# supernomad/quantum

Measured on AMD Instinct MI355X. Metric: AES-256-GCM seal+unseal GiB/s (device-resident packets) at 1/2/4/8 MI355X, higher is better.
Workload: dtype u8

## Files before the change

### quantum_amd/csrc/gcm_kernels.hip

```cpp
#include <hip/hip_runtime.h>
#include <stdint.h>

#include <algorithm>

#include "gcm_internal.h"

namespace qgcm {

typedef __attribute__((address_space(3))) uint32_t lds_u32;
typedef uint32_t u32x4 __attribute__((ext_vector_type(4)));
typedef __attribute__((address_space(3))) u32x4 lds_u128;

struct __attribute__((aligned(4))) W4 {
    uint32_t x, y, z, w;
};

#ifndef QGCM_NT_DATA
#define QGCM_NT_DATA 0
#endif
typedef uint32_t u32x4u __attribute__((ext_vector_type(4), aligned(4)));
__device__ __forceinline__ W4 load_block(const W4 *p) {
    if constexpr ((QGCM_NT_DATA & 1) != 0) {
        const u32x4u v = __builtin_nontemporal_load(reinterpret_cast<const u32x4u *>(p));
        return W4{v.x, v.y, v.z, v.w};
// ... 415 lines not shown
__device__ __forceinline__ void write_tail(uint8_t *data, uint32_t L, uint32_t g0, uint32_t g1, uint32_t g2,
                                           uint32_t g3, uint32_t n0, uint32_t n1, uint32_t n2, uint32_t prefix) {
    const uint32_t s = L & 3u;
    uint32_t *t = reinterpret_cast<uint32_t *>(data + (L & ~3u));
    const uint32_t sh = 32 - 8 * s;
    t[0] = (uint32_t)((((uint64_t)g0 << 32) | ((uint64_t)prefix << sh)) >> sh);
    t[1] = funnel(g1, g0, sh);
    t[2] = funnel(g2, g1, sh);
    t[3] = funnel(g3, g2, sh);
    t[4] = funnel(n0, g3, sh);
    t[5] = funnel(n1, n0, sh);
    t[6] = funnel(n2, n1, sh);
    if (s) store_bytes(data + (L & ~3u) + 28, n2 >> sh, s);
}

__device__ __forceinline__ uint32_t quad_xor(uint32_t v) {
    v ^= (uint32_t)__builtin_amdgcn_mov_dpp((int)v, 0xB1, 0xf, 0xf, false);
    v ^= (uint32_t)__builtin_amdgcn_mov_dpp((int)v, 0x4E, 0xf, 0xf, false);
    return v;
}

template <bool kSeal, class Eng>
__device__ __forceinline__ void quad_packet(const Batch &b, const Eng &eng, uint32_t pkt, uint64_t off, uint32_t L,
                                            uint32_t wkey, uint32_t m, uint32_t gH4) {
    const uint4 *Hg = b.gh_table + (size_t)wkey * kGhEntries;
    uint8_t *raw = b.arena + off;
    uint8_t *data = raw + 4;

    uint32_t g0 = 0, g1 = 0, g2 = 0, g3 = 0, n0, n1, n2;
    if (kSeal && b.nonces) {
        const uint32_t *np = reinterpret_cast<const uint32_t *>(b.nonces + 12ull * pkt);
        n0 = np[0];
        n1 = np[1];
        n2 = np[2];
    } else {
        read_nonce(data, L, n0, n1, n2);
    }
    const uint32_t nfull = L >> 4, r = L & 15u;
    const uint32_t d = nfull + (r ? 1u : 0u);

    uint32_t z0 = 0, z1 = 0, z2 = 0, z3 = 0;
    if (m == 3 && b.aad_len)
        z0 = *reinterpret_cast<const uint32_t *>(raw) & (b.aad_len >= 4 ? 0xffffffffu : lowmask(b.aad_len));
    int blast = -1;

    uint32_t e0 = 0, e1 = 0, e2 = 0, e3 = 0;
    uint32_t prefix = 0;
    {
    Ctr cc;
    uint32_t hi = 0;
    eng.setup(cc, n0, n1, n2, 0);
    for (uint32_t bi = m; bi < nfull; bi += 4) {
        const uint32_t ctr = bi + 2;
        if ((ctr >> 8) != hi) {
            hi = ctr >> 8;
            eng.setup(cc, n0, n1, n2, hi);
        }
        W4 *p = reinterpret_cast<W4 *>(data + 16u * bi);
        const W4 in = load_block(p);
        uint32_t k0, k1, k2, k3;
        eng.block(cc, ctr & 0xffu, k0, k1, k2, k3);
        const W4 out = {in.x ^ k0, in.y ^ k1, in.z ^ k2, in.w ^ k3};
        store_block(p, out);
        const W4 &c = kSeal ? out : in;
        eng.ghash(z0, z1, z2, z3, gH4);
        z0 ^= c.x;
        z1 ^= c.y;
        z2 ^= c.z;
        z3 ^= c.w;
        blast = (int)bi;
    }
    const bool part = r && (nfull & 3u) == m;
    if (part || m == (d & 3u)) {
        const uint32_t ctr = part ? nfull + 2 : 1u;
        if ((ctr >> 8) != hi) {
            hi = ctr >> 8;
            eng.setup(cc, n0, n1, n2, hi);
        }
        uint32_t k0, k1, k2, k3;
        eng.block(cc, ctr & 0xffu, k0, k1, k2, k3);
        if (part) {
            uint8_t *blk = data + 16u * nfull;
            const W4 in = *reinterpret_cast<const W4 *>(blk);
            const uint32_t q = r >> 2, sb = r & 3u;
            const uint32_t o0 = in.x ^ k0, o1 = in.y ^ k1, o2 = in.z ^ k2, o3 = in.w ^ k3;
            uint32_t *bw = reinterpret_cast<uint32_t *>(blk);
            if (q > 0) bw[0] = o0;
            if (q > 1) bw[1] = o1;
            if (q > 2) bw[2] = o2;
            const uint32_t oq = sel4(q, o0, o1, o2, o3) & lowmask(sb);
            W4 c = kSeal ? W4{o0, o1, o2, o3} : in;
            if (kSeal)
                prefix = oq;
            else
                store_bytes(blk + 4 * q, oq, sb);
            c.x &= q > 0 ? 0xffffffffu : lowmask(sb);
            c.y &= q > 1 ? 0xffffffffu : (q == 1 ? lowmask(sb) : 0u);
            c.z &= q > 2 ? 0xffffffffu : (q == 2 ? lowmask(sb) : 0u);
            c.w &= q == 3 ? lowmask(sb) : 0u;
            eng.ghash(z0, z1, z2, z3, gH4);
            z0 ^= c.x;
            z1 ^= c.y;
            z2 ^= c.z;
            z3 ^= c.w;
            blast = (int)nfull;
        } else {
            e0 = k0;
            e1 = k1;
            e2 = k2;
            e3 = k3;
        }
    }
    }
    {
        const uint32_t em = d + 1u - (uint32_t)blast;
        const uint32_t tsel = em == 2 ? kGhH2 : em == 3 ? kGhH3 : em == 4 ? kGhH4 : kGhH5;
        ghash_mul_global(z0, z1, z2, z3, Hg + tsel);
        uint32_t l0, l1, l2, l3;
        ghash_lenblock_global(b.aad_len, L, Hg, l0, l1, l2, l3);
        z0 = quad_xor(z0) ^ l0;
        z1 = quad_xor(z1) ^ l1;
        z2 = quad_xor(z2) ^ l2;
        z3 = quad_xor(z3) ^ l3;
    }
    e0 = quad_xor(e0);
    e1 = quad_xor(e1);
    e2 = quad_xor(e2);
    e3 = quad_xor(e3);
    const uint32_t t0 = z0 ^ e0, t1 = z1 ^ e1, t2 = z2 ^ e2, t3 = z3 ^ e3;
    const uint32_t owner = r ? (nfull & 3u) : 0u;
    if (kSeal) {
        if (m == owner) {
            write_tail(data, L, t0, t1, t2, t3, n0, n1, n2, prefix);
            if (b.status) b.status[pkt] = 1;
        }
    } else {
        read_tag(data, L, g0, g1, g2, g3);
        const bool ok = ((t0 ^ g0) | (t1 ^ g1) | (t2 ^ g2) | (t3 ^ g3)) == 0;
        if (!ok) {
            for (uint32_t bi = m; bi < nfull; bi += 4) {
                const W4 zz = {0, 0, 0, 0};
                *reinterpret_cast<W4 *>(data + 16u * bi) = zz;
            }
            if (r && m == owner) {
                uint32_t *bw = reinterpret_cast<uint32_t *>(data + 16u * nfull);
                for (uint32_t w = 0; w < (r >> 2); ++w) bw[w] = 0;
                store_bytes(data + 16u * nfull + (r & ~3u), 0, r & 3u);
            }
        }
        if (b.status && m == 0) b.status[pkt] = ok ? 1 : 0;
    }
}

#ifndef QGCM_TILE_POOL
#define QGCM_TILE_POOL 4
#endif
#ifndef QGCM_TAIL_EIGHTHS
#define QGCM_TAIL_EIGHTHS 4
#endif
constexpr uint32_t kPoolCtr = kG5Bytes + kTeBytes;

#ifdef QGCM_QUAD_STATS
__device__ unsigned long long g_quad_stats[4096 * 8];
#endif

template <bool kDesc>
constexpr int quad_waves() { return kDesc ? 12 : 16; }
template <bool kDesc>
constexpr int quad_wpe() { return kDesc ? 3 : 8; }

template <bool kSeal, bool kDesc>
__global__ void __launch_bounds__(quad_waves<kDesc>() * 64) __attribute__((amdgpu_waves_per_eu(quad_wpe<kDesc>(),
                                                                                                  quad_wpe<kDesc>())))
gcm_quad_kernel(Batch b, const uint32_t *__restrict__ rk_table) {
    constexpr uint32_t kW = quad_waves<kDesc>();
    constexpr uint32_t kT = kW * 64;
    constexpr uint32_t kTeBase = kDesc ? 0u : kG5Bytes;
    const uint32_t lane = threadIdx.x & 63u;
    const uint32_t wave = threadIdx.x >> 6;
    const uint32_t m = lane & 3u;
    const uint32_t qd = lane >> 2;
    if (kDesc && b.tile_list && __builtin_amdgcn_readfirstlane(*b.n_list) == 0) return;

    for (uint32_t i = threadIdx.x; i < kTeBytes / 4; i += kT) {
        const uint32_t x = i >> 6, slot = i & 63u;
        lds_st32(kTeBase + 4 * i, b.te[(slot >> 5) * 256u + x]);
    }
    if constexpr (!kDesc) g5_fill(b.gh_table + (size_t)b.uniform_key * kGhEntries + kGhH4, threadIdx.x, kT);
    if constexpr (!kDesc && QGCM_TILE_POOL) {
        if (threadIdx.x == 0) lds_st32(kPoolCtr, kW);
    }
#if QGCM_TILE_POOL == 4
    if constexpr (!kDesc) {
        if (threadIdx.x == 0) lds_st32(kPoolCtr + 12, 0u);
    }
#endif
    __syncthreads();

    const uint32_t lb = (lane & 31u) << 2;
    const uint32_t m8 = vreg(0x0000ff00u), mf8 = vreg(0x000000f8u);
    const uint32_t gH4 = kDesc ? kTeBytes + wave * kGhBytes : 0u;
    uint32_t cur_key = kDesc ? 0xffffffffu : b.uniform_key;
    const uint32_t ntiles = kDesc ? (b.tile_list ? *b.n_list : b.n_items >> 4) : ((b.n + 15) >> 4);

#ifdef QGCM_QUAD_STATS
    unsigned long long *qs = g_quad_stats + (size_t)blockIdx.x * 8u;
    uint32_t qs_tiles = 0;
    if (!kDesc && threadIdx.x == 0) {
        qs[0] = wall_clock64();
        qs[4] = __builtin_amdgcn_s_getreg((31 << 11) | 20);
        qs[5] = __builtin_amdgcn_s_getreg((31 << 11) | 4);
    }
#endif
#ifdef QGCM_QUAD_STATS
#define QS_TILE() ++qs_tiles
#define QS_END()                                                  \
    do {                                                          \
        if (!kDesc && lane == 0) {                                \
            const unsigned long long t_ = wall_clock64();         \
            atomicMax(&qs[1], t_);                                \
            atomicAdd(&qs[2], t_);                                \
            atomicAdd(&qs[3], (unsigned long long)qs_tiles);      \
            atomicMax(&qs[6], (1ull << 62) - t_);                 \
        }                                                         \
    } while (0)
#else
#define QS_TILE() do { } while (0)
#define QS_END() do { } while (0)
#endif
#if QGCM_TILE_POOL == 4
    uint32_t sidx = 0xffffffffu, tail0 = 0;
    if constexpr (!kDesc) {
        const uint32_t rows = ntiles / (gridDim.x * kW);
        if (b.pool && rows > 0) {
            const uint32_t tail_rows = rows < 2 ? 0u : std::min(rows - 1u, std::max(1u, rows * QGCM_TAIL_EIGHTHS / 8u));
            sidx = (rows - tail_rows) * kW;
            tail0 = (rows - tail_rows) * gridDim.x * kW;
        }
    }
#endif
    uint32_t tile = blockIdx.x * kW + wave;
    if constexpr (kDesc) {
        uint32_t t = 0;
        if (lane == 0) t = atomicAdd(b.tile_counter, 1u);
        tile = __builtin_amdgcn_readfirstlane(__shfl(t, 0));
    }
    for (; tile < ntiles;) {
        uint32_t pkt, L;
        bool valid;
        uint64_t off;
        uint32_t wkey = cur_key;
        if constexpr (kDesc) {
            const uint32_t wt = b.tile_list ? b.tile_list[tile] : tile;
            pkt = b.worklist[wt * 16u + qd];
            valid = pkt != 0xffffffffu;
            qgcm_desc dsc = {0, 0, 0};
            if (valid) dsc = b.descs[pkt];
            off = dsc.offset;
            L = kSeal ? dsc.len : dsc.len - QGCM_OVERHEAD;
            const uint64_t vmask = __ballot(valid);
            if (vmask != 0) {
                wkey = __builtin_amdgcn_readfirstlane(__shfl(dsc.key_idx, __ffsll((unsigned long long)vmask) - 1));
                if (wkey != cur_key) {
                    const uint4 *src = b.gh_table + (size_t)wkey * kGhEntries + kGhH4;
#pragma unroll
                    for (int r = 0; r < 8; ++r) {
                        const uint32_t e = r * 64 + lane;
                        lds_st_comb(gH4, e, src[e]);
                    }
                    __builtin_amdgcn_fence(__ATOMIC_RELEASE, "wavefront");
                    __builtin_amdgcn_wave_barrier();
                    __builtin_amdgcn_fence(__ATOMIC_ACQUIRE, "wavefront");
                    cur_key = wkey;
                }
            }
            uint32_t t = 0;
            if (lane == 0) t = atomicAdd(b.tile_counter, 1u);
            const uint32_t next = __builtin_amdgcn_readfirstlane(__shfl(t, 0));
            asm volatile("" : "+v"(L));
            if (!valid) {
                tile = next;
                continue;
            }
            tile = next;
        } else {
            pkt = tile * 16u + qd;
            L = b.uniform_len;
            asm volatile("" : "+s"(L));
            valid = pkt < b.n;
            if (!kSeal) {
                if (L < (uint32_t)QGCM_OVERHEAD) valid = false;
                L -= QGCM_OVERHEAD;
            }
            off = (uint64_t)pkt * b.stride;
            if constexpr (QGCM_TILE_POOL) {
                uint32_t i = 0;
                if (lane == 0) i = __atomic_fetch_add((lds_u32 *)(size_t)kPoolCtr, 1u, __ATOMIC_RELAXED);
                i = __builtin_amdgcn_readfirstlane(i);
                tile = blockIdx.x * kW + (i % kW) + (i / kW) * gridDim.x * kW;
#if QGCM_TILE_POOL == 4
                if (i >= sidx) {
                    uint32_t c = 0;
                    if (lane == 0) c = atomicAdd(b.pool, 1u);
                    tile = tail0 + __builtin_amdgcn_readfirstlane(c);
                }
#endif
            } else {
                tile += gridDim.x * kW;
            }
            if (!valid) {
                if (!kSeal && b.status && pkt < b.n && m == 0) b.status[pkt] = 0;
                continue;
            }
        }
        const Keys kk = {rk_table + (size_t)wkey * kRkWords, rk_table + (size_t)wkey * kRkWords + 64};
        if constexpr (kDesc) {
            quad_packet<kSeal>(b, Tab2{kk, {lb, m8}}, pkt, off, L, wkey, m, gH4);
        } else {
            quad_packet<kSeal>(b, Tab2F{kk, {lb, m8}, mf8}, pkt, off, L, wkey, m, gH4);
        }
        QS_TILE();
    }
    QS_END();
#if QGCM_TILE_POOL == 4
    if constexpr (!kDesc) {
        if (b.pool) {
            uint32_t last = 0;
            if (lane == 0 && __atomic_fetch_add((lds_u32 *)(size_t)(kPoolCtr + 12), 1u, __ATOMIC_RELAXED) == kW - 1) {
                __threadfence();
                last = atomicAdd(b.pool + kPoolDoneWord, 1u) == gridDim.x - 1u ? 1u : 0u;
            }
            if (lane == 0 && last) {
                __threadfence();
                b.pool[0] = 0;
                b.pool[kPoolDoneWord] = 0;
                __threadfence_system();
                __hip_atomic_store(b.pool_done, b.pool_gen, __ATOMIC_RELEASE, __HIP_MEMORY_SCOPE_SYSTEM);
            }
        }
    }
#endif
}
#undef QS_TILE
#undef QS_END

#ifdef QGCM_QUAD_STATS
extern "C" int qgcm_debug_quad_stats(unsigned long long *out, int n, int reset) {
    if (n > 4096 * 8) n = 4096 * 8;
    if (hipMemcpyFromSymbol(out, HIP_SYMBOL(g_quad_stats), (size_t)n * 8) != hipSuccess) return -1;
    if (reset) {
        static unsigned long long zero[4096 * 8];
        if (hipMemcpyToSymbol(HIP_SYMBOL(g_quad_stats), zero, sizeof(zero)) != hipSuccess) return -1;
    }
    return 0;
}
#endif

constexpr uint32_t kSegCtl = kG5Bytes + kTeBytes;
constexpr uint32_t kSegLds = kSegCtl + 16u;
constexpr uint32_t kSegDone = 0xffffffffu;

__device__ __forceinline__ volatile lds_u32 *seg_ctl(uint32_t i) { return (volatile lds_u32 *)(size_t)(kSegCtl + 4u * i); }

template <class P>
__device__ __forceinline__ uint32_t wave_lower_bound(uint32_t lo, uint32_t hi, uint32_t lane, P pred) {
    while (hi - lo > 63u) {
        const uint32_t step = (hi - lo + 62u) / 63u;
        const uint32_t p = min(lo + lane * step, hi);
        const uint64_t msk = __ballot(pred(p));
        const uint32_t f = (uint32_t)__ffsll((unsigned long long)msk) - 1u;
        if (f == 0) return lo;
        const uint32_t nlo = lo + (f - 1u) * step + 1u, nhi = min(lo + f * step, hi);
        lo = nlo;
        hi = nhi;
    }
    const uint64_t msk = __ballot(pred(min(lo + lane, hi)));
    return lo + (uint32_t)__ffsll((unsigned long long)msk) - 1u;
}

#ifdef QGCM_SEG_STATS
__device__ unsigned long long g_seg_stats[4096 * 16];
#define SEG_STAT_ADD(i, v) \
    do { if (lane == 0) atomicAdd(&g_seg_stats[blockIdx.x * 16u + (i)], (unsigned long long)(v)); } while (0)
#define SEG_NOW() wall_clock64()
#else
#define SEG_STAT_ADD(i, v) do { } while (0)
#define SEG_NOW() 0ull
#endif

#ifndef QGCM_SEG_START
#define QGCM_SEG_START 1
#endif
#ifndef QGCM_SEG_HELP_MIN
#define QGCM_SEG_HELP_MIN 16
#endif
#ifndef QGCM_SEG_LAST
#define QGCM_SEG_LAST 0
#endif
__device__ __forceinline__ void seg_next_phase(const Batch &b, uint32_t &r, uint32_t nruns, bool &helping,
                                               uint32_t lane) {
    uint32_t found = kSegDone;
    if (!helping) {
        uint32_t c = 0;
        if (lane == 0) c = atomicAdd(b.tile_counter, 1u);
        c = __builtin_amdgcn_readfirstlane(__shfl(c, 0));
        if (c < nruns)
            found = c;
        else
            helping = true;
    }
    if (helping) {
        if (QGCM_SEG_START) {
            const uint32_t h = (blockIdx.x * 0x9E3779B1u) ^ (r * 0x85EBCA6Bu + 0x632BE5ABu);
            r = (uint32_t)(((uint64_t)(h ^ (h >> 15)) * nruns) >> 32);
        }
        for (uint32_t pass = 0, need = QGCM_SEG_HELP_MIN; pass < (QGCM_SEG_LAST ? 2u : 1u) && found == kSegDone;
             ++pass, need = QGCM_SEG_LAST ? QGCM_SEG_LAST : 1u)
        for (uint32_t base = 0; base < nruns; base += 256u) {
            bool left[4];
            uint32_t idx[4];
#pragma unroll
            for (uint32_t j = 0; j < 4; ++j) {
                const uint32_t o = base + 64u * j + lane;
                uint32_t i = r + o;
                i = i >= nruns ? i - nruns : i;
                idx[j] = i;
                left[j] = false;
                if (o < nruns) {
                    const uint2 run = b.runs[i];
                    left[j] = __hip_atomic_load(b.run_next + i, __ATOMIC_RELAXED, __HIP_MEMORY_SCOPE_AGENT) +
                                  need <= run.y - run.x;
                }
            }
#pragma unroll
            for (uint32_t j = 0; j < 4 && found == kSegDone; ++j) {
                const uint64_t msk = __ballot(left[j]);
                if (msk) found = __builtin_amdgcn_readfirstlane(__shfl(idx[j], (int)__ffsll((unsigned long long)msk) - 1));
            }
            if (found != kSegDone) break;
        }
    }
    uint32_t key = kSegDone;
    if (found != kSegDone) {
        r = found;
        key = b.tile_keys[b.runs[found].x];
    }
    if (lane == 0) {
        *seg_ctl(0) = found;
        *seg_ctl(1) = key;
    }
}

#ifndef QGCM_SEG_CLAIM
#define QGCM_SEG_CLAIM 1
#endif

template <bool kSeal>
__global__ void __launch_bounds__(1024) __attribute__((amdgpu_waves_per_eu(8, 8)))
gcm_seg_kernel(Batch b, const uint32_t *__restrict__ rk_table) {
    constexpr uint32_t kT = 1024;
    const uint32_t lane = threadIdx.x & 63u;
    const uint32_t wave = threadIdx.x >> 6;
    const uint32_t m = lane & 3u;
    const uint32_t qd = lane >> 2;
    if (__builtin_amdgcn_readfirstlane(*b.nruns) == 0) return;
    for (uint32_t i = threadIdx.x; i < kTeBytes / 4; i += kT) {
        const uint32_t x = i >> 6, slot = i & 63u;
        lds_st32(kG5Bytes + 4 * i, b.te[(slot >> 5) * 256u + x]);
    }
    const uint32_t lb = (lane & 31u) << 2;
    const uint32_t m8 = vreg(0x0000ff00u), mf8 = vreg(0x000000f8u);
    const uint32_t ntiles = b.n_items >> 4;
    uint32_t table_key = kSegDone;
    uint32_t r = 0, nruns = 0;
// ... 1274 lines not shown
```

### quantum_amd/csrc/qgcm_api.cpp

```cpp
#include <hip/hip_runtime.h>
#include <errno.h>
#include <stdint.h>
#include <stdio.h>
#include <stdlib.h>
#include <string.h>
#include <sys/random.h>

#include <algorithm>
#include <atomic>
#include <chrono>
#include <memory>
#include <future>
#include <map>
#include <mutex>
#include <thread>
#include <vector>

#include "../../include/qgcm.h"
#include "chain_claim.h"
#include "gcm_internal.h"
#include "kdf_core.h"

using namespace qgcm;

constexpr int kPipeStreams = 3;
constexpr uint64_t kPipeChunk = 32ull << 20;
constexpr uint64_t kHostChunk = 64ull << 20;
constexpr uint64_t kHostRing = 4ull << 30;

struct qgcm_ctx {
    int device = 0;
    int num_cus = 0;
    uint32_t max_keys = 0;
    int uniform_variant = kVariantUniform;
    int desc_variant = kVariantDescQuad;
    int wgs_per_cu_override = 0;
    bool one_kernel = true;
    bool variant_forced = false;
    uint32_t desc_one_max = kDescOneMax;
    uint32_t direct_max = kDirectMax;
    uint32_t one_uniform_max = kOneUniformMax;
    uint32_t launch_chunk = kLaunchChunk;
    uint32_t desc_chunk = kDescChunk;
    bool desc_one_on = true, host_direct = true, small_wl = true;
    uint64_t chain_chunk = kPipeChunk;
    int chain_slots = kPipeStreams, chain_dev_ahead = 2, chain_dev_backlog = -1;
    bool snappy_group = true;
    int snappy_per_cu = 0;
    bool chain_pin = true;
    std::mutex codec_cpus_mu;
    std::vector<int> codec_cpus;
    uint32_t *d_rk = nullptr;
    uint4 *d_gh = nullptr;
    uint4 *d_pw = nullptr;
    uint32_t pw_keys = 0;
    uint32_t *d_te = nullptr;
    uint8_t *d_sbox = nullptr;
    uint8_t *d_key_valid = nullptr;
    std::vector<uint8_t> key_set;
    std::mutex key_mu;

    std::mutex ws_mu;
    void *d_qws = nullptr;
    size_t qws_cap = 0;

    std::mutex io_mu;
    struct OneSlot {
        std::mutex mu;
        hipStream_t stream = nullptr;
        uint8_t *h = nullptr;
        size_t cap = 0;
    };
    static constexpr int kOneSlots = 8;
    static constexpr size_t kOneSlotCap = kOneCap + 4096;
    static_assert((kOneCap - 16u) + 16u <= kOneSlotCap, "record, tail and status bytes fit a pooled staging slot");
    static_assert(one_fits_launch(16336, true, QGCM_MAX_AAD) && !one_fits_launch(16337, true, QGCM_MAX_AAD) &&
                      one_record_bytes(16336, true) + one_tail_bytes(QGCM_MAX_AAD) + 16u <= kOneSlotCap,
                  "the largest long-AAD call fits a pooled staging slot");
    OneSlot one[kOneSlots];
    OneSlot big;
    std::atomic<uint32_t> one_rr{0};

    hipStream_t pipe[kPipeStreams] = {};
    std::vector<hipEvent_t> ev_in, ev_kern, ev_out;
    uint64_t host_chunk = kHostChunk, host_ring = kHostRing;
    uint8_t *d_ring = nullptr;
    size_t ring_cap = 0;
    uint8_t *h_stat = nullptr;
    size_t hstat_cap = 0;
    uint8_t *d_side = nullptr;
    size_t side_cap = 0;
    qgcm_desc *h_desc = nullptr;
    uint32_t *h_lens = nullptr;
    std::vector<hipStream_t> chain_extra;
    size_t hdesc_cap = 0;

    hipEvent_t ws_done = nullptr;
    bool ws_pending = false;

    uint32_t *d_pool = nullptr;
    uint32_t *h_pool_done = nullptr;
    uint32_t pool_gen[kPoolSets] = {};
    uint32_t pool_launches = 0;
    uint32_t pool_sets = kPoolSets;
    std::mutex pool_mu;

    qgcm::NonceRng rng;

    std::atomic<uint64_t> launches[QGCM_KERNEL_COUNTERS] = {};
    void count(int k, uint64_t v = 1) { launches[k].fetch_add(v, std::memory_order_relaxed); }

    std::atomic<int> chain_codec{1};

    bool res_on = true;
    qgcm::ResidentConfig res_cfg{};
    std::atomic<qgcm::Resident *> res{nullptr};
    std::atomic<bool> res_failed{false};
    std::mutex res_mu;

    uint32_t kdf_device_min = kKdfDeviceMin;
    std::mutex kdf_mu;
    hipStream_t kdf_stream = nullptr;
    std::atomic<uint64_t> kdf_stats[4] = {};
    std::atomic<uint64_t> ecdh_stats[3] = {};

    qgcm::RouteState *route = nullptr;
};

namespace {

thread_local bool tl_dummy;

int env_int(const char *name, int dflt) {
    const char *v = getenv(name);
    return v && *v ? atoi(v) : dflt;
}

uint8_t gf8_mul(uint8_t a, uint8_t b) {
    uint8_t p = 0;
    for (int i = 0; i < 8; ++i) {
        if (b & 1) p ^= a;
        const uint8_t hi = a & 0x80;
        a <<= 1;
        if (hi) a ^= 0x1b;
        b >>= 1;
    }
    return p;
}

void build_tables(uint8_t sbox[256], uint32_t te[512]) {
    for (int x = 0; x < 256; ++x) {
        uint8_t inv = 0;
        if (x) {
            uint8_t r = 1, b = (uint8_t)x;
            for (int e = 254; e; e >>= 1) {
                if (e & 1) r = gf8_mul(r, b);
                b = gf8_mul(b, b);
            }
            inv = r;
        }
        auto rl = [](uint8_t v, int s) { return (uint8_t)((v << s) | (v >> (8 - s))); };
        sbox[x] = inv ^ rl(inv, 1) ^ rl(inv, 2) ^ rl(inv, 3) ^ rl(inv, 4) ^ 0x63;
    }
    for (int x = 0; x < 256; ++x) {
        const uint32_t s = sbox[x], s2 = gf8_mul((uint8_t)s, 2), s3 = s2 ^ s;
        const uint32_t t0 = s2 | (s << 8) | (s << 16) | (s3 << 24);
        te[x] = t0;
        te[256 + x] = (t0 << 8) | (t0 >> 24);
    }
}

void set_err(char *err, int errlen, const char *msg) {
    if (err && errlen > 0) snprintf(err, (size_t)errlen, "%s", msg);
}

int hip_fail(hipError_t e) { return e == hipSuccess ? QGCM_OK : QGCM_E_HIP; }

int grid_for(const qgcm_ctx *ctx, uint32_t n_items, int variant) {
    const int cus = std::max(1, ctx->num_cus - resident_workers_running(ctx->res.load(std::memory_order_acquire)));
    const uint32_t waves = (uint32_t)variant_waves(variant);
    const uint32_t tiles = (n_items + 15) / 16;
    const uint32_t wgs = (tiles + waves - 1) / waves;
    const uint32_t per_cu = ctx->wgs_per_cu_override > 0 ? (uint32_t)ctx->wgs_per_cu_override
                                                         : (uint32_t)variant_wgs_per_cu(variant);
    const uint32_t cap = (uint32_t)cus * per_cu;
    return (int)(wgs < cap ? (wgs ? wgs : 1) : cap);
}

Batch base_batch(const qgcm_ctx *ctx) {
    Batch b{};
    b.rk_table = ctx->d_rk;
    b.gh_table = ctx->d_gh;
    b.pw_table = ctx->d_pw;
    b.pw_keys = ctx->pw_keys;
    b.te = ctx->d_te;
    b.key_valid = ctx->d_key_valid;
    b.max_keys = ctx->max_keys;
    return b;
}

int run_uniform(qgcm_ctx *ctx, bool seal, uint8_t *arena, uint64_t stride, uint32_t n, uint32_t len,
                uint32_t key_idx, const uint8_t *nonces, uint32_t aad_len, uint8_t *status, hipStream_t s,
                const NonceLease *lease = nullptr, uint64_t lease_pos = 0);

inline bool generate(const uint8_t *nonces) { return nonces == QGCM_NONCES_GENERATE; }

int nonce_launch(qgcm_ctx *ctx, NonceDest dest, const NonceLease &l, uint8_t *out, const qgcm_desc *descs,
                 uint64_t stride, uint32_t len, uint32_t n, bool one, hipStream_t s) {
    NonceArgs a{};
    a.keys = l.keys;
    a.v0 = l.v[0];
    a.v1 = l.v[1];
    a.v2 = l.v[2];
    a.v3 = l.v[3];
    a.out = out;
    a.descs = descs;
    a.key_valid = ctx->d_key_valid;
    a.te = ctx->d_te;
    a.stride = stride;
    a.len = len;
    a.n = n;
    a.max_keys = ctx->max_keys;
    a.one = one ? 1u : 0u;
    return hip_fail(launch_nonce_fill(dest, a, ctx->num_cus, s));
}

int run_one(qgcm_ctx *ctx, bool seal, uint8_t *slot, uint64_t stride, uint32_t len, uint32_t key_idx,
            uint32_t aad_len, uint8_t *status, hipStream_t s) {
    if (ctx->one_kernel && stride + one_tail_bytes(aad_len) <= kOneCap - 16 && !(stride & 15) &&
        !((uintptr_t)slot & 15)) {
        volatile uint8_t *done = status + 1;
        *done = 0;
        Batch b = base_batch(ctx);
        b.done = status + 1;
        b.arena = slot;
        b.status = status;
        b.stride = stride;
        b.uniform_len = len;
        b.uniform_key = key_idx;
        b.n = 1;
        b.n_items = 64;
        b.aad_len = aad_len;
        if (launch_one(seal, b, s) != hipSuccess) return QGCM_E_HIP;
        ctx->count(QGCM_KERNEL_ONE);
        const auto t0 = std::chrono::steady_clock::now();
        for (uint32_t spins = 0; *done == 0; ++spins) {
            __builtin_ia32_pause();
            if ((spins & 1023) == 1023 && std::chrono::steady_clock::now() - t0 > std::chrono::seconds(1)) break;
        }
        if (*done == 0) return hip_fail(hipStreamSynchronize(s));
        std::atomic_thread_fence(std::memory_order_acquire);
        return QGCM_OK;
    }
    if (aad_len > 4) return QGCM_E_ARG;
    const int rc = run_uniform(ctx, seal, slot, stride, 1, len, key_idx, nullptr, aad_len, status, s);
    return rc == QGCM_OK ? hip_fail(hipStreamSynchronize(s)) : rc;
}

Resident *get_resident(qgcm_ctx *ctx) {
    Resident *r = ctx->res.load(std::memory_order_acquire);
    if (r || !ctx->res_on || ctx->res_failed.load(std::memory_order_relaxed)) return r;
    std::lock_guard<std::mutex> g(ctx->res_mu);
    r = ctx->res.load(std::memory_order_acquire);
    if (!r) {
        r = resident_create(ctx->device, base_batch(ctx), ctx->num_cus, ctx->res_cfg);
        if (!r) ctx->res_failed = true;
        ctx->res.store(r, std::memory_order_release);
    }
    return r;
}

bool key_ok(qgcm_ctx *ctx, uint32_t k) {
    if (k >= ctx->max_keys) return false;
    return __atomic_load_n(&ctx->key_set[k], __ATOMIC_ACQUIRE) != 0;
}

}

bool qgcm::ctx_one_kernel(const qgcm_ctx *ctx) { return ctx->one_kernel; }
hipStream_t qgcm::ctx_pipe(qgcm_ctx *ctx, int k) { return ctx->pipe[k]; }
std::mutex &qgcm::ctx_io_mu(qgcm_ctx *ctx) { return ctx->io_mu; }
qgcm::RouteState *qgcm::ctx_route(qgcm_ctx *ctx) { return ctx->route; }
uint32_t qgcm::ctx_max_keys(const qgcm_ctx *ctx) { return ctx->max_keys; }
int qgcm::ctx_device(const qgcm_ctx *ctx) { return ctx->device; }
int qgcm::ctx_num_cus(const qgcm_ctx *ctx) { return ctx->num_cus; }

uint32_t qgcm::descs_one_max(const qgcm_ctx *ctx) {
    return ctx->one_kernel && !ctx->variant_forced && ctx->desc_one_on ? ctx->desc_one_max : 0u;
}

uint64_t qgcm::pinned_view(const void *p, uint64_t bytes) {
    hipPointerAttribute_t a;
    if (hipPointerGetAttributes(&a, p) != hipSuccess || a.type != hipMemoryTypeHost || !a.devicePointer) {
        (void)hipGetLastError();
        return 0;
    }
    hipDeviceptr_t base = nullptr;
    size_t size = 0;
    if (hipMemGetAddressRange(&base, &size, a.devicePointer) != hipSuccess || !base) {
        (void)hipGetLastError();
        return 0;
    }
    const uint64_t dv = reinterpret_cast<uint64_t>(a.devicePointer), b = reinterpret_cast<uint64_t>(base);
    return dv >= b && dv + bytes <= b + size ? dv : 0;
}

uint32_t qgcm::direct_max(const qgcm_ctx *ctx) { return descs_one_max(ctx) ? ctx->direct_max : 0u; }

int qgcm::run_descs_one(qgcm_ctx *ctx, bool seal, uint8_t *d_arena, const qgcm_desc *d_descs, uint32_t n,
                        const uint8_t *d_nonces, uint32_t aad_len, uint8_t *d_status, hipStream_t s) {
    if (!ctx || !n || !d_arena || !d_descs || aad_len > 4 || n > QGCM_MAX_BATCH || !descs_one_max(ctx) ||
        ((uintptr_t)d_arena & 15))
        return QGCM_E_ARG;
    if (hipSetDevice(ctx->device) != hipSuccess) return QGCM_E_HIP;
    if (seal && generate(d_nonces)) {
        NonceLease l;
        if (!ctx->rng.reserve(n, l)) return QGCM_E_NOMEM;
        const int rc = nonce_launch(ctx, kNonceDescs, l, d_arena, d_descs, 0, 0, n, true, s);
        if (rc != QGCM_OK) return rc;
        d_nonces = nullptr;
    }
    Batch b = base_batch(ctx);
    b.arena = d_arena;
    b.descs = d_descs;
    b.nonces = seal ? d_nonces : nullptr;
    b.status = d_status;
    b.n = n;
    b.n_items = (n + 63) & ~63u;
    b.aad_len = aad_len;
    if (launch_one(seal, b, s) != hipSuccess) return QGCM_E_HIP;
    ctx->count(QGCM_KERNEL_ONE);
    return QGCM_OK;
}

namespace {

int run_uniform(qgcm_ctx *ctx, bool seal, uint8_t *arena, uint64_t stride, uint32_t n, uint32_t len,
                uint32_t key_idx, const uint8_t *nonces, uint32_t aad_len, uint8_t *status, hipStream_t s,
// ... 288 lines not shown
    std::lock_guard<std::mutex> lk(ctx->kdf_mu);
    hipStream_t s = kdf_stream_locked(ctx);
    if (!s) return QGCM_E_HIP;
    const size_t bytes = (size_t)count * 32;
    uint8_t *d_in = nullptr;
    const size_t in_bytes = 2 * bytes + (pp ? 64 : 0);
    if (hipMalloc(&d_in, in_bytes) != hipSuccess) return QGCM_E_NOMEM;
    uint32_t launches = 0, ladder_launches = 0;
    int rc = QGCM_OK;
    if (pp) {
        secrets = pp->pub_keys;
        salts = pp->pub_salts;
    }
    if (hipMemcpyAsync(d_in, secrets, bytes, hipMemcpyHostToDevice, s) != hipSuccess ||
        hipMemcpyAsync(d_in + bytes, salts, bytes, hipMemcpyHostToDevice, s) != hipSuccess)
        rc = QGCM_E_HIP;
    if (rc == QGCM_OK && pp &&
        (hipMemcpyAsync(d_in + 2 * bytes, pp->priv_key, 32, hipMemcpyHostToDevice, s) != hipSuccess ||
         hipMemcpyAsync(d_in + 2 * bytes + 32, pp->priv_salt, 32, hipMemcpyHostToDevice, s) != hipSuccess ||
         launch_x25519(d_in + 2 * bytes, 0, d_in, 2 * count, d_in, count, s, &ladder_launches) != hipSuccess))
        rc = QGCM_E_HIP;
    if (rc == QGCM_OK && launch_kdf(d_in, d_in + bytes, count, iters, d_keys, s, &launches) != hipSuccess) rc = QGCM_E_HIP;
    if (hipMemsetAsync(d_in, 0, in_bytes, s) != hipSuccess) rc = QGCM_E_HIP;
    if (h_out) {
        if (rc == QGCM_OK && hipMemcpyAsync(h_out, d_keys, bytes, hipMemcpyDeviceToHost, s) != hipSuccess) rc = QGCM_E_HIP;
        if (hipMemsetAsync(d_keys, 0, bytes, s) != hipSuccess) rc = QGCM_E_HIP;
    }
    if (hipStreamSynchronize(s) != hipSuccess) rc = QGCM_E_HIP;
    hipFree(d_in);
    ctx->kdf_stats[2].fetch_add(launches, std::memory_order_relaxed);
    ctx->ecdh_stats[2].fetch_add(ladder_launches, std::memory_order_relaxed);
    if (rc == QGCM_OK) {
        ctx->kdf_stats[0].fetch_add(count, std::memory_order_relaxed);
        if (pp) ctx->ecdh_stats[0].fetch_add(2ull * count, std::memory_order_relaxed);
    }
    return rc;
}

void wipe_device_keys(qgcm_ctx *ctx, uint8_t *d_keys, uint32_t count) {
    std::lock_guard<std::mutex> lk(ctx->kdf_mu);
    hipStream_t s = ctx->kdf_stream;
    if (hipMemsetAsync(d_keys, 0, (size_t)count * 32, s) == hipSuccess) (void)hipStreamSynchronize(s);
}

}

int qgcm::derive_install_runs(qgcm_ctx *ctx, const KeyRun *runs, size_t nruns, uint32_t count, const uint8_t *secrets,
                              const uint8_t *salts, const PeerPublics *pp) {
    if (count == 0) return QGCM_OK;
    if (hipSetDevice(ctx->device) != hipSuccess) return QGCM_E_HIP;
    uint8_t *d_keys = nullptr;
    if (hipMalloc(&d_keys, (size_t)count * 32) != hipSuccess) return QGCM_E_NOMEM;
    int rc;
    if (ctx->kdf_device_min && count >= ctx->kdf_device_min) {
        rc = kdf_on_device(ctx, secrets, salts, count, QGCM_PBKDF2_ITERS, d_keys, nullptr, pp);
        if (rc == QGCM_OK) rc = install_device_keys(ctx, runs, nruns, d_keys, count, nullptr);
        else wipe_device_keys(ctx, d_keys, count);
    } else {
        std::vector<uint8_t> keys((size_t)count * 32), shared;
        rc = QGCM_OK;
        if (pp) {
            shared.resize((size_t)count * 64);
            rc = qgcm_x25519_batch(pp->priv_key, 0, pp->pub_keys, count, shared.data());
            if (rc == QGCM_OK) rc = qgcm_x25519_batch(pp->priv_salt, 0, pp->pub_salts, count, shared.data() + (size_t)count * 32);
            if (rc == QGCM_OK) ctx->ecdh_stats[1].fetch_add(2ull * count, std::memory_order_relaxed);
            secrets = shared.data();
            salts = shared.data() + (size_t)count * 32;
        }
        if (rc == QGCM_OK) rc = qgcm_derive_keys(secrets, salts, count, keys.data());
        if (!shared.empty()) explicit_bzero(shared.data(), shared.size());
        if (rc == QGCM_OK) {
            ctx->kdf_stats[1].fetch_add(count, std::memory_order_relaxed);
            rc = install_device_keys(ctx, runs, nruns, d_keys, count, keys.data());
        }
        explicit_bzero(keys.data(), keys.size());
    }
    hipFree(d_keys);
    return rc;
}

extern "C" {

const char *qgcm_version(void) { return "qgcm 0.1.0 (gfx950)"; }

int qgcm_device_count(void) {
    int n = 0;
    if (hipGetDeviceCount(&n) != hipSuccess) {
        (void)hipGetLastError();
        return 0;
    }
    return n;
}

const char *qgcm_strerror(int code) {
    switch (code) {
        case QGCM_OK: return "ok";
        case QGCM_E_ARG: return "invalid argument";
        case QGCM_E_HIP: return "HIP runtime error";
        case QGCM_E_KEY: return "key index not set or out of range";
        case QGCM_E_AUTH: return "message authentication failed";
        case QGCM_E_NOMEM: return "out of device or pinned memory";
        default: return "unknown error";
    }
}

qgcm_ctx *qgcm_create(int device, uint32_t max_keys, char *err, int errlen) {
    (void)tl_dummy;
    if (max_keys == 0 || max_keys > QGCM_MAX_KEYS) {
        set_err(err, errlen, "max_keys must be in [1, 2^20 - 1]");
        return nullptr;
    }
    int ndev = 0;
    if (hipGetDeviceCount(&ndev) != hipSuccess || device < 0 || device >= ndev) {
        set_err(err, errlen, "no such HIP device");
        return nullptr;
    }
    if (hipSetDevice(device) != hipSuccess) {
        set_err(err, errlen, "hipSetDevice failed");
        return nullptr;
    }
    hipDeviceProp_t prop;
    if (hipGetDeviceProperties(&prop, device) != hipSuccess) {
        set_err(err, errlen, "hipGetDeviceProperties failed");
        return nullptr;
    }
    if (strncmp(prop.gcnArchName, "gfx950", 6) != 0) {
        char m[QGCM_ERRLEN];
        snprintf(m, sizeof m, "device %d is %s; libqgcm is built for gfx950 only", device, prop.gcnArchName);
        set_err(err, errlen, m);
        return nullptr;
    }
    {
        static std::mutex init_mu;
        std::lock_guard<std::mutex> g(init_mu);
        if (init_kernels() != hipSuccess) {
            set_err(err, errlen, "kernel setup failed");
            return nullptr;
        }
    }
    auto *ctx = new qgcm_ctx();
    ctx->device = device;
    ctx->num_cus = prop.multiProcessorCount;
    ctx->max_keys = max_keys;
    ctx->key_set.assign(max_keys, 0);
    ctx->route = route_state_create();
    if (const char *v = getenv("QGCM_VARIANT")) {
        const int iv = atoi(v);
        if (variant_valid(iv) && !variant_desc(iv)) {
            ctx->uniform_variant = iv;
            ctx->variant_forced = true;
        }
    }
    if (const char *v = getenv("QGCM_WGS_PER_CU")) ctx->wgs_per_cu_override = atoi(v);
    if (const char *v = getenv("QGCM_ONE_KERNEL")) ctx->one_kernel = atoi(v) != 0;
    if (const char *v = getenv("QGCM_CHAIN_DEVICE")) ctx->chain_codec = std::max(0, std::min(2, atoi(v)));
    if (const char *v = getenv("QGCM_RESIDENT")) ctx->res_on = atoi(v) != 0;
    ctx->res_cfg = qgcm::resident_config_from_env();
    if (const char *v = getenv("QGCM_ONE_UNIFORM_MAX")) ctx->one_uniform_max = (uint32_t)std::max(0, atoi(v));
    if (const char *v = getenv("QGCM_DESC_ONE_MAX")) ctx->desc_one_max = (uint32_t)std::max(0, atoi(v));
    if (const char *v = getenv("QGCM_DIRECT_MAX")) ctx->direct_max = (uint32_t)std::max(0, atoi(v));
    if (const char *v = getenv("QGCM_LAUNCH_CHUNK"))
        ctx->launch_chunk = (uint32_t)std::max(0, atoi(v)) & ~63u;
    if (const char *v = getenv("QGCM_DESC_CHUNK")) ctx->desc_chunk = (uint32_t)std::max(0, atoi(v));
    if (const char *v = getenv("QGCM_PIPE_CHUNK_MB")) ctx->host_chunk = (uint64_t)std::max(1, atoi(v)) << 20;
    if (const char *v = getenv("QGCM_PIPE_RING_MB")) ctx->host_ring = (uint64_t)std::max(1, atoi(v)) << 20;
    if (const char *v = getenv("QGCM_NONCE_RESEED"))
        ctx->rng.set_interval(std::max<uint64_t>(1, strtoull(v, nullptr, 0)));
    if (const char *v = getenv("QGCM_DESC_VARIANT")) {
        const int iv = atoi(v);
        if (variant_valid(iv) && variant_desc(iv)) ctx->desc_variant = iv;
    }
    auto off = [](const char *name) {
        const char *v = getenv(name);
        return v && !strcmp(v, "0");
    };
    ctx->chain_chunk = (uint64_t)std::max(1, env_int("QGCM_CHAIN_CHUNK_MB", (int)(kPipeChunk >> 20))) << 20;
    ctx->chain_slots = std::max(1, std::min(16, env_int("QGCM_CHAIN_SLOTS", kPipeStreams)));
    ctx->chain_dev_ahead = std::max(1, env_int("QGCM_CHAIN_DEV_AHEAD", 2));
    ctx->chain_dev_backlog = env_int("QGCM_CHAIN_DEV_BACKLOG", -1);
    ctx->snappy_group = env_int("QGCM_SNAPPY_GROUP", 1) != 0;
    ctx->snappy_per_cu = std::max(0, env_int("QGCM_SNAPPY_PER_CU", 0));
    ctx->chain_pin = env_int("QGCM_CHAIN_PIN", 1) != 0;
    ctx->desc_one_on = !off("QGCM_DESC_ONE");
    ctx->host_direct = !off("QGCM_HOST_DIRECT");
    ctx->small_wl = !off("QGCM_SMALL_WORKLIST");
    ctx->kdf_device_min = (uint32_t)std::max(0, env_int("QGCM_KDF_DEVICE_MIN", (int)kKdfDeviceMin));
    uint8_t sbox[256];
    uint32_t te[512];
    build_tables(sbox, te);
    bool ok = hipMalloc(&ctx->d_rk, (size_t)max_keys * kRkWords * 4) == hipSuccess &&
              hipMalloc(&ctx->d_gh, (size_t)max_keys * kGhEntries * 16) == hipSuccess &&
              hipMalloc(&ctx->d_key_valid, max_keys) == hipSuccess &&
              hipMemset(ctx->d_rk, 0, (size_t)max_keys * kRkWords * 4) == hipSuccess &&
              hipMemset(ctx->d_gh, 0, (size_t)max_keys * kGhEntries * 16) == hipSuccess &&
              hipMemset(ctx->d_key_valid, 0, max_keys) == hipSuccess &&
              hipMalloc(&ctx->d_te, sizeof te) == hipSuccess && hipMalloc(&ctx->d_sbox, sizeof sbox) == hipSuccess &&
              hipMemcpy(ctx->d_te, te, sizeof te, hipMemcpyHostToDevice) == hipSuccess &&
              hipMemcpy(ctx->d_sbox, sbox, sizeof sbox, hipMemcpyHostToDevice) == hipSuccess &&
              hipEventCreateWithFlags(&ctx->ws_done, hipEventDisableTiming) == hipSuccess;
    ctx->pw_keys = (uint32_t)std::min<int64_t>(max_keys, std::max(0, env_int("QGCM_FLAT_GHASH_KEYS", 256)));
    if (ok && ctx->pw_keys &&
        (hipMalloc(&ctx->d_pw, (size_t)ctx->pw_keys * kPwPowers * kPwEntries * 16) != hipSuccess ||
         hipMemset(ctx->d_pw, 0, (size_t)ctx->pw_keys * kPwPowers * kPwEntries * 16) != hipSuccess)) {
        hipFree(ctx->d_pw);
        ctx->d_pw = nullptr;
        ctx->pw_keys = 0;
    }
    for (int k = 0; ok && k < kPipeStreams; ++k)
        ok = hipStreamCreateWithFlags(&ctx->pipe[k], hipStreamNonBlocking) == hipSuccess;
    ctx->pool_sets = (uint32_t)std::max(1, std::min((int)kPoolSets, env_int("QGCM_POOL_SETS", (int)kPoolSets)));
    if (ok && quad_pool_global()) {
        const size_t bytes = (size_t)kPoolSets * kPoolSetWords * 4;
        ok = hipMalloc(&ctx->d_pool, bytes) == hipSuccess && hipMemset(ctx->d_pool, 0, bytes) == hipSuccess &&
             hipHostMalloc(&ctx->h_pool_done, kPoolSets * 4, hipHostMallocCoherent | hipHostMallocMapped) ==
                 hipSuccess;
        if (ok) memset(ctx->h_pool_done, 0, kPoolSets * 4);
    }
    if (!ok) {
        set_err(err, errlen, "device allocation / kernel setup failed");
        qgcm_destroy(ctx);
        return nullptr;
    }
    if (ctx->chain_pin) (void)codec_cpu_list(ctx->device);
    return ctx;
}

void qgcm_destroy(qgcm_ctx *ctx) {
    if (!ctx) return;
    resident_destroy(ctx->res.exchange(nullptr));
    hipSetDevice(ctx->device);
    hipDeviceSynchronize();
    hipFree(ctx->d_rk);
    hipFree(ctx->d_gh);
    hipFree(ctx->d_pw);
    hipFree(ctx->d_te);
    hipFree(ctx->d_sbox);
    hipFree(ctx->d_key_valid);
    hipFree(ctx->d_qws);
    route_state_destroy(ctx->route);
    auto free_slot = [](qgcm_ctx::OneSlot &sl) {
        if (sl.h) hipHostFree(sl.h);
        if (sl.stream) hipStreamDestroy(sl.stream);
    };
    for (auto &sl : ctx->one) free_slot(sl);
    free_slot(ctx->big);
    hipFree(ctx->d_ring);
    hipFree(ctx->d_side);
    if (ctx->h_stat) hipHostFree(ctx->h_stat);
    if (ctx->h_desc) hipHostFree(ctx->h_desc);
    if (ctx->h_lens) hipHostFree(ctx->h_lens);
    for (hipStream_t x : ctx->chain_extra) hipStreamDestroy(x);
    if (ctx->kdf_stream) hipStreamDestroy(ctx->kdf_stream);
    for (hipStream_t p : ctx->pipe)
        if (p) hipStreamDestroy(p);
    if (ctx->ws_done) hipEventDestroy(ctx->ws_done);
    hipFree(ctx->d_pool);
    if (ctx->h_pool_done) hipHostFree(ctx->h_pool_done);
    for (auto *v : {&ctx->ev_in, &ctx->ev_kern, &ctx->ev_out})
        for (hipEvent_t e : *v) hipEventDestroy(e);
    delete ctx;
}

int qgcm_set_keys(qgcm_ctx *ctx, uint32_t first_idx, uint32_t count, const uint8_t *keys) {
    if (!ctx || (count && !keys)) return QGCM_E_ARG;
    if ((uint64_t)first_idx + count > ctx->max_keys) return QGCM_E_KEY;
    if (count == 0) return QGCM_OK;
    if (hipSetDevice(ctx->device) != hipSuccess) return QGCM_E_HIP;
    uint8_t *d_keys = nullptr;
    if (hipMalloc(&d_keys, (size_t)count * 32) != hipSuccess) return QGCM_E_NOMEM;
    const KeyRun run{first_idx, count, 0};
    const int rc = install_device_keys(ctx, &run, 1, d_keys, count, keys);
    hipFree(d_keys);
    return rc;
}

int qgcm_set_key(qgcm_ctx *ctx, uint32_t key_idx, const uint8_t key[QGCM_KEY_BYTES]) {
    return qgcm_set_keys(ctx, key_idx, 1, key);
}

int qgcm_derive_keys_device(qgcm_ctx *ctx, const uint8_t *secrets, const uint8_t *salts, uint32_t count, uint32_t iters,
                            uint8_t *keys) {
    if (!ctx || (count && (!secrets || !salts || !keys))) return QGCM_E_ARG;
    if (count == 0) return QGCM_OK;
    if (iters == 0 || iters > kKdfMaxIters) return QGCM_E_ARG;
    if (hipSetDevice(ctx->device) != hipSuccess) return QGCM_E_HIP;
    uint8_t *d_keys = nullptr;
    if (hipMalloc(&d_keys, (size_t)count * 32) != hipSuccess) return QGCM_E_NOMEM;
    std::vector<uint8_t> out((size_t)count * 32);
    const int rc = kdf_on_device(ctx, secrets, salts, count, iters, d_keys, out.data());
    hipFree(d_keys);
    if (rc == QGCM_OK) memcpy(keys, out.data(), out.size());
    explicit_bzero(out.data(), out.size());
    return rc;
}

int qgcm_derive_set_keys(qgcm_ctx *ctx, uint32_t first_idx, uint32_t count, const uint8_t *secrets,
                         const uint8_t *salts) {
    if (!ctx || (count && (!secrets || !salts))) return QGCM_E_ARG;
    if ((uint64_t)first_idx + count > ctx->max_keys) return QGCM_E_KEY;
    if (count == 0) return QGCM_OK;
    const KeyRun run{first_idx, count, 0};
    return derive_install_runs(ctx, &run, 1, count, secrets, salts);
}

int qgcm_x25519_batch(const uint8_t *scalars, uint32_t scalar_stride, const uint8_t *points, uint32_t count,
                      uint8_t *out) {
// ... 836 lines not shown
```

Before: 848.0.

## Split uniform quad kernel into main pass and deferred two-tile tail/tag pass

In the uniform (non-descriptor) quad kernel, the per-packet work now has two parts. The main pass does the full-block CTR and GHASH work. The tail pass covers the partial block, the length block, tag encryption and verify, and is deferred so that two tiles' tails run together. Lanes m<2 handle the current tile's tail and lanes m>=2 handle the held tile's, and DPP broadcasts and swaps exchange the GHASH partial sums. This is meant to spread the serial tail work across all four lanes of a quad instead of leaving lanes idle. The cost is more complex control flow and extra register pressure. An optional env cap on the quad grid size is also added; it is off by default.

```diff
diff --git a/quantum_amd/csrc/gcm_kernels.hip b/quantum_amd/csrc/gcm_kernels.hip
--- a/quantum_amd/csrc/gcm_kernels.hip
+++ b/quantum_amd/csrc/gcm_kernels.hip
@@ -591,6 +591,171 @@
     }
 }
 
+__device__ __forceinline__ uint32_t quad_bcast(uint32_t v, uint32_t j) {
+    const int x = (int)v;
+    return (uint32_t)(j == 0   ? __builtin_amdgcn_mov_dpp(x, 0x00, 0xf, 0xf, false)
+                      : j == 1 ? __builtin_amdgcn_mov_dpp(x, 0x55, 0xf, 0xf, false)
+                      : j == 2 ? __builtin_amdgcn_mov_dpp(x, 0xAA, 0xf, 0xf, false)
+                               : __builtin_amdgcn_mov_dpp(x, 0xFF, 0xf, 0xf, false));
+}
+__device__ __forceinline__ uint32_t pair_swap(uint32_t v) {
+    return (uint32_t)__builtin_amdgcn_mov_dpp((int)v, 0xB1, 0xf, 0xf, false);
+}
+
+template <bool kSeal>
+__device__ __forceinline__ uint32_t quad_main(const Batch &b, const Tab2F &eng, uint32_t pkt, uint64_t off, uint32_t L,
+                                              uint32_t m, const uint4 *Hg) {
+    uint8_t *raw = b.arena + off;
+    uint8_t *data = raw + 4;
+    uint32_t n0, n1, n2;
+    if (kSeal && b.nonces) {
+        const uint32_t *np = reinterpret_cast<const uint32_t *>(b.nonces + 12ull * pkt);
+        n0 = np[0];
+        n1 = np[1];
+        n2 = np[2];
+    } else {
+        read_nonce(data, L, n0, n1, n2);
+    }
+    const uint32_t nfull = L >> 4;
+    const uint32_t d = nfull + ((L & 15u) ? 1u : 0u);
+    uint32_t z0 = 0, z1 = 0, z2 = 0, z3 = 0;
+    if (m == 3 && b.aad_len)
+        z0 = *reinterpret_cast<const uint32_t *>(raw) & (b.aad_len >= 4 ? 0xffffffffu : lowmask(b.aad_len));
+    int blast = -1;
+    Ctr cc;
+    uint32_t hi = 0;
+    eng.setup(cc, n0, n1, n2, 0);
+    for (uint32_t it = 0, bi = m; bi < nfull; bi += 4, ++it) {
+        const uint32_t ctr = bi + 2;
+        if ((ctr >> 8) != hi) {
+            hi = ctr >> 8;
+            eng.setup(cc, n0, n1, n2, hi);
+        }
+        W4 *p = reinterpret_cast<W4 *>(data + 16u * bi);
+        const W4 in = load_block(p);
+        uint32_t k0, k1, k2, k3;
+        eng.block(cc, ctr & 0xffu, k0, k1, k2, k3);
+        const W4 out = {in.x ^ k0, in.y ^ k1, in.z ^ k2, in.w ^ k3};
+        store_block(p, out);
+        const W4 &c = kSeal ? out : in;
+        if (it == 0) {
+            if (b.aad_len) {
+                const uint32_t y[4] = {z0, z1, z2, z3};
+                z0 = z1 = z2 = z3 = 0;
+                g5_chunk<0, 7>(y, eng.mf8, z0, z1, z2, z3);
+            }
+        } else {
+            eng.ghash(z0, z1, z2, z3, 0u);
+        }
+        z0 ^= c.x;
+        z1 ^= c.y;
+        z2 ^= c.z;
+        z3 ^= c.w;
+        blast = (int)bi;
+    }
+    const uint32_t em = d - (uint32_t)blast;
+    const uint32_t tsel = em == 1 ? kGhH : em == 2 ? kGhH2 : em == 3 ? kGhH3 : em == 4 ? kGhH4 : kGhH5;
+    ghash_mul_global(z0, z1, z2, z3, Hg + tsel);
+    return sel4(m, quad_xor(z0), quad_xor(z1), quad_xor(z2), quad_xor(z3));
+}
+
+constexpr uint32_t kNoTile = 0xffffffffu;
+template <bool kSeal>
+__device__ __forceinline__ void quad_tails(const Batch &b, const Tab2F &eng, uint32_t cur, uint32_t held,
+                                           uint32_t acur, uint32_t aheld, uint32_t L, uint32_t m, uint32_t qd,
+                                           const uint4 *Hg) {
+    const bool second = m >= 2;
+    const bool j0 = (m & 1u) != 0;
+    uint32_t v0, v1, v2, v3;
+    {
+        const uint32_t c0 = quad_bcast(acur, 0), c1 = quad_bcast(acur, 1), c2 = quad_bcast(acur, 2);
+        const uint32_t c3 = quad_bcast(acur, 3);
+        const uint32_t h0 = quad_bcast(aheld, 0), h1 = quad_bcast(aheld, 1), h2 = quad_bcast(aheld, 2);
+        const uint32_t h3 = quad_bcast(aheld, 3);
+        v0 = second ? h0 : c0;
+        v1 = second ? h1 : c1;
+        v2 = second ? h2 : c2;
+        v3 = second ? h3 : c3;
+    }
+    const uint32_t tile = second ? held : cur;
+    const uint32_t pkt = tile * 16u + qd;
+    if (tile == kNoTile || pkt >= b.n) return;
+    uint8_t *data = b.arena + (uint64_t)pkt * b.stride + 4;
+    uint32_t n0, n1, n2;
+    if (kSeal && b.nonces) {
+        const uint32_t *np = reinterpret_cast<const uint32_t *>(b.nonces + 12ull * pkt);
+        n0 = np[0];
+        n1 = np[1];
+        n2 = np[2];
+    } else {
+        read_nonce(data, L, n0, n1, n2);
+    }
+    const uint32_t nfull = L >> 4, r = L & 15u;
+    const uint32_t ctr = j0 ? 1u : nfull + 2;
+    uint32_t k0, k1, k2, k3;
+    {
+        Ctr cc;
+        eng.setup(cc, n0, n1, n2, ctr >> 8);
+        eng.block(cc, ctr & 0xffu, k0, k1, k2, k3);
+    }
+    uint32_t prefix = 0;
+    if (j0) {
+        v1 ^= bswap(b.aad_len * 8u);
+        v3 ^= bswap(L * 8u);
+    } else {
+        v0 = v1 = v2 = v3 = 0;
+        if (r) {
+            uint8_t *blk = data + 16u * nfull;
+            const W4 in = *reinterpret_cast<const W4 *>(blk);
+            const uint32_t q = r >> 2, sb = r & 3u;
+            const uint32_t o0 = in.x ^ k0, o1 = in.y ^ k1, o2 = in.z ^ k2, o3 = in.w ^ k3;
+            uint32_t *bw = reinterpret_cast<uint32_t *>(blk);
+            if (q > 0) bw[0] = o0;
+            if (q > 1) bw[1] = o1;
+            if (q > 2) bw[2] = o2;
+            const uint32_t oq = sel4(q, o0, o1, o2, o3) & lowmask(sb);
+            if (kSeal)
+                prefix = oq;
+            else
+                store_bytes(blk + 4 * q, oq, sb);
+            v0 = (kSeal ? o0 : in.x) & (q > 0 ? 0xffffffffu : lowmask(sb));
+            v1 = (kSeal ? o1 : in.y) & (q > 1 ? 0xffffffffu : (q == 1 ? lowmask(sb) : 0u));
+            v2 = (kSeal ? o2 : in.z) & (q > 2 ? 0xffffffffu : (q == 2 ? lowmask(sb) : 0u));
+            v3 = (kSeal ? o3 : in.w) & (q == 3 ? lowmask(sb) : 0u);
+        }
+    }
+    ghash_mul_global(v0, v1, v2, v3, Hg + (j0 ? kGhH : kGhH2));
+    if (j0) {
+        v0 ^= k0;
+        v1 ^= k1;
+        v2 ^= k2;
+        v3 ^= k3;
+    }
+    const uint32_t t0 = v0 ^ pair_swap(v0), t1 = v1 ^ pair_swap(v1), t2 = v2 ^ pair_swap(v2), t3 = v3 ^ pair_swap(v3);
+    if (kSeal) {
+        if (!j0) {
+            write_tail(data, L, t0, t1, t2, t3, n0, n1, n2, prefix);
+            if (b.status) b.status[pkt] = 1;
+        }
+    } else {
+        uint32_t g0, g1, g2, g3;
+        read_tag(data, L, g0, g1, g2, g3);
+        const bool ok = ((t0 ^ g0) | (t1 ^ g1) | (t2 ^ g2) | (t3 ^ g3)) == 0;
+        if (!ok) {
+            for (uint32_t bi = m & 1u; bi < nfull; bi += 2) {
+                const W4 zz = {0, 0, 0, 0};
+                *reinterpret_cast<W4 *>(data + 16u * bi) = zz;
+            }
+            if (r && !j0) {
+                uint32_t *bw = reinterpret_cast<uint32_t *>(data + 16u * nfull);
+                for (uint32_t w = 0; w < (r >> 2); ++w) bw[w] = 0;
+                store_bytes(data + 16u * nfull + (r & ~3u), 0, r & 3u);
+            }
+        }
+        if (b.status && !j0) b.status[pkt] = ok ? 1 : 0;
+    }
+}
+
 #ifndef QGCM_TILE_POOL
 #define QGCM_TILE_POOL 4
 #endif
@@ -684,12 +849,12 @@
         if (lane == 0) t = atomicAdd(b.tile_counter, 1u);
         tile = __builtin_amdgcn_readfirstlane(__shfl(t, 0));
     }
-    for (; tile < ntiles;) {
-        uint32_t pkt, L;
-        bool valid;
-        uint64_t off;
-        uint32_t wkey = cur_key;
-        if constexpr (kDesc) {
+    if constexpr (kDesc) {
+        for (; tile < ntiles;) {
+            uint32_t pkt, L;
+            bool valid;
+            uint64_t off;
+            uint32_t wkey = cur_key;
             const uint32_t wt = b.tile_list ? b.tile_list[tile] : tile;
             pkt = b.worklist[wt * 16u + qd];
             valid = pkt != 0xffffffffu;
@@ -722,43 +887,54 @@
                 continue;
             }
             tile = next;
-        } else {
-            pkt = tile * 16u + qd;
-            L = b.uniform_len;
+            const Keys kk = {rk_table + (size_t)wkey * kRkWords, rk_table + (size_t)wkey * kRkWords + 64};
+            quad_packet<kSeal>(b, Tab2{kk, {lb, m8}}, pkt, off, L, wkey, m, gH4);
+        }
+    } else {
+        const uint4 *Hg = b.gh_table + (size_t)cur_key * kGhEntries;
+        const Keys kk = {rk_table + (size_t)cur_key * kRkWords, rk_table + (size_t)cur_key * kRkWords + 64};
+        const Tab2F eng{kk, {lb, m8}, mf8};
+        uint32_t held = kNoTile, aheld = 0;
+        for (;;) {
+            const bool have = tile < ntiles;
+            if (!have && held == kNoTile) break;
+            uint32_t L = b.uniform_len;
             asm volatile("" : "+s"(L));
-            valid = pkt < b.n;
-            if (!kSeal) {
-                if (L < (uint32_t)QGCM_OVERHEAD) valid = false;
-                L -= QGCM_OVERHEAD;
-            }
-            off = (uint64_t)pkt * b.stride;
-            if constexpr (QGCM_TILE_POOL) {
-                uint32_t i = 0;
-                if (lane == 0) i = __atomic_fetch_add((lds_u32 *)(size_t)kPoolCtr, 1u, __ATOMIC_RELAXED);
-                i = __builtin_amdgcn_readfirstlane(i);
-                tile = blockIdx.x * kW + (i % kW) + (i / kW) * gridDim.x * kW;
+            if (!kSeal) L -= QGCM_OVERHEAD;
+            uint32_t cur = kNoTile, acur = 0;
+            if (have) {
+                cur = tile;
+                const uint32_t pkt = tile * 16u + qd;
+                if constexpr (QGCM_TILE_POOL) {
+                    uint32_t i = 0;
+                    if (lane == 0) i = __atomic_fetch_add((lds_u32 *)(size_t)kPoolCtr, 1u, __ATOMIC_RELAXED);
+                    i = __builtin_amdgcn_readfirstlane(i);
+                    tile = blockIdx.x * kW + (i % kW) + (i / kW) * gridDim.x * kW;
 #if QGCM_TILE_POOL == 4
-                if (i >= sidx) {
-                    uint32_t c = 0;
-                    if (lane == 0) c = atomicAdd(b.pool, 1u);
-                    tile = tail0 + __builtin_amdgcn_readfirstlane(c);
+                    if (i >= sidx) {
+                        uint32_t c = 0;
+                        if (lane == 0) c = atomicAdd(b.pool, 1u);
+                        tile = tail0 + __builtin_amdgcn_readfirstlane(c);
+                    }
+#endif
+                } else {
+                    tile += gridDim.x * kW;
                 }
-#endif
+                if (!kSeal && b.uniform_len < (uint32_t)QGCM_OVERHEAD) {
+                    if (b.status && pkt < b.n && m == 0) b.status[pkt] = 0;
+                    continue;
+                }
+                if (pkt < b.n) acur = quad_main<kSeal>(b, eng, pkt, (uint64_t)pkt * b.stride, L, m, Hg);
+                QS_TILE();
+            }
+            if (held != kNoTile) {
+                quad_tails<kSeal>(b, eng, cur, held, acur, aheld, L, m, qd, Hg);
+                held = kNoTile;
             } else {
-                tile += gridDim.x * kW;
-            }
-            if (!valid) {
-                if (!kSeal && b.status && pkt < b.n && m == 0) b.status[pkt] = 0;
-                continue;
-            }
-        }
-        const Keys kk = {rk_table + (size_t)wkey * kRkWords, rk_table + (size_t)wkey * kRkWords + 64};
-        if constexpr (kDesc) {
-            quad_packet<kSeal>(b, Tab2{kk, {lb, m8}}, pkt, off, L, wkey, m, gH4);
-        } else {
-            quad_packet<kSeal>(b, Tab2F{kk, {lb, m8}, mf8}, pkt, off, L, wkey, m, gH4);
-        }
-        QS_TILE();
+                held = cur;
+                aheld = acur;
+            }
+        }
     }
     QS_END();
 #if QGCM_TILE_POOL == 4
diff --git a/quantum_amd/csrc/qgcm_api.cpp b/quantum_amd/csrc/qgcm_api.cpp
--- a/quantum_amd/csrc/qgcm_api.cpp
+++ b/quantum_amd/csrc/qgcm_api.cpp
@@ -35,6 +35,7 @@
     int uniform_variant = kVariantUniform;
     int desc_variant = kVariantDescQuad;
     int wgs_per_cu_override = 0;
+    int quad_grid_cap = 0;
     bool one_kernel = true;
     bool variant_forced = false;
     uint32_t desc_one_max = kDescOneMax;
@@ -183,7 +184,8 @@
     const uint32_t wgs = (tiles + waves - 1) / waves;
     const uint32_t per_cu = ctx->wgs_per_cu_override > 0 ? (uint32_t)ctx->wgs_per_cu_override
                                                          : (uint32_t)variant_wgs_per_cu(variant);
-    const uint32_t cap = (uint32_t)cus * per_cu;
+    uint32_t cap = (uint32_t)cus * per_cu;
+    if (ctx->quad_grid_cap > 0 && !variant_desc(variant)) cap = std::min(cap, (uint32_t)ctx->quad_grid_cap);
     return (int)(wgs < cap ? (wgs ? wgs : 1) : cap);
 }
 
@@ -778,6 +780,7 @@
         }
     }
     if (const char *v = getenv("QGCM_WGS_PER_CU")) ctx->wgs_per_cu_override = atoi(v);
+    if (const char *v = getenv("QGCM_QUAD_GRID")) ctx->quad_grid_cap = std::max(0, atoi(v));
     if (const char *v = getenv("QGCM_ONE_KERNEL")) ctx->one_kernel = atoi(v) != 0;
     if (const char *v = getenv("QGCM_CHAIN_DEVICE")) ctx->chain_codec = std::max(0, std::min(2, atoi(v)));
     if (const char *v = getenv("QGCM_RESIDENT")) ctx->res_on = atoi(v) != 0;
```

Measured after the change: 856.3 (median of 6 runs). Within noise of the previous version (+1.0%).
